# cloudflare/zkp-ecdsa

Measured on NVIDIA H100. Metric: ZKAttest proofs/sec, higher is better.
Workload: dtype u256/u258 (32-bit limbs, Montgomery)

## Files before the change

zkp_ecdsa_b200/csrc/zk_ops.cuh:

```cuda
#pragma once
#include "zk_curves.cuh"
#include "zk_layout.h"
#include "zk_sha256.cuh"

namespace zk {

#if defined(__CUDA_ARCH__)
#define ZK_SET_STATUS(ptr, code) atomicCAS((int*)(ptr), 0, (int)(code))
#define ZK_POST_MIN(ptr, key) atomicMin((int*)(ptr), (int)(key))
#define ZK_SET_STATUS_OVER(ptr, code, over) \
  do {                                      \
    atomicCAS((int*)(ptr), 0, (int)(code)); \
    atomicCAS((int*)(ptr), (int)(over), (int)(code)); \
  } while (0)
#else
#define ZK_SET_STATUS_OVER(ptr, code, over)              \
  do {                                                   \
    if (*(ptr) == 0 || *(ptr) == (over)) *(ptr) = (code); \
  } while (0)
#define ZK_SET_STATUS(ptr, code) \
  do {                           \
    if (*(ptr) == 0) *(ptr) = (code); \
  } while (0)
#define ZK_POST_MIN(ptr, key)             \
  do {                                    \
    if ((int)(key) < *(ptr)) *(ptr) = (int)(key); \
  } while (0)
#endif

template <int N>
ZK_HD void ld(uint32_t* r, const uint32_t* p) {
#pragma unroll
  for (int i = 0; i < N; i++) r[i] = p[i];
}
template <int N>
ZK_HD void st(uint32_t* p, const uint32_t* r) {
#pragma unroll
  for (int i = 0; i < N; i++) p[i] = r[i];
}

enum : int {
  P256_PROJ_WORDS = 24,
  P256_AFF_WORDS = 16,
#if defined(ZKA_PG_WAR256)
  TOM_PROJ_WORDS = 24,
  TOM_E2_WORDS = 24,
  TOM_AFF_WORDS = 16,
  TOM_PRE_WORDS = 16,
#else
  TOM_PROJ_WORDS = 28,
  TOM_E2_WORDS = 36,
  TOM_AFF_WORDS = 18,
  TOM_PRE_WORDS = 32,
#endif
  NORM_CHUNK_MAX = 64,
};


#if defined(ZKA_PG_WAR256)
ZK_HD void tom_st_xyz(uint32_t* m, const uint32_t* x, const uint32_t* y, const uint32_t* z) {
  st<8>(m, x); st<8>(m + 8, y); st<8>(m + 16, z);
}
ZK_HD void tom_ld_xyz(uint32_t* x, uint32_t* y, uint32_t* z, const uint32_t* m) {
  ld<8>(x, m); ld<8>(y, m + 8); ld<8>(z, m + 16);
}
ZK_HD void tom_ld_pre(TomPre& q, const uint32_t* m) { ld<8>(q.x, m); ld<8>(q.y, m + 8); }
#else
ZK_HD void tom_st_xyz(uint32_t* m, const uint32_t* x, const uint32_t* y, const uint32_t* z) {
  uint32_t w[28];
#pragma unroll
  for (int i = 0; i < 9; i++) { w[i] = x[i]; w[9 + i] = y[i]; w[18 + i] = z[i]; }
  w[27] = 0;
#if defined(__CUDA_ARCH__)
  uint4* v = reinterpret_cast<uint4*>(m);
#pragma unroll
  for (int i = 0; i < 7; i++) v[i] = make_uint4(w[4 * i], w[4 * i + 1], w[4 * i + 2], w[4 * i + 3]);
#else
  for (int i = 0; i < 28; i++) m[i] = w[i];
#endif
}
ZK_HD void tom_ld_xyz(uint32_t* x, uint32_t* y, uint32_t* z, const uint32_t* m) {
  uint32_t w[28];
#if defined(__CUDA_ARCH__)
  const uint4* v = reinterpret_cast<const uint4*>(m);
#pragma unroll
  for (int i = 0; i < 7; i++) {
    const uint4 u = v[i];
    w[4 * i] = u.x; w[4 * i + 1] = u.y; w[4 * i + 2] = u.z; w[4 * i + 3] = u.w;
  }
#else
  for (int i = 0; i < 28; i++) w[i] = m[i];
#endif
#pragma unroll
  for (int i = 0; i < 9; i++) { x[i] = w[i]; y[i] = w[9 + i]; z[i] = w[18 + i]; }
}
ZK_HD void tom_st_efgh(uint32_t* m, const TomEfgh& p) {
  uint32_t w[36];
#pragma unroll
  for (int i = 0; i < 9; i++) { w[i] = p.e[i]; w[9 + i] = p.f[i]; w[18 + i] = p.g[i]; w[27 + i] = p.h[i]; }
#if defined(__CUDA_ARCH__)
  uint4* v = reinterpret_cast<uint4*>(m);
#pragma unroll
  for (int i = 0; i < 9; i++) v[i] = make_uint4(w[4 * i], w[4 * i + 1], w[4 * i + 2], w[4 * i + 3]);
#else
  for (int i = 0; i < 36; i++) m[i] = w[i];
#endif
}
ZK_HD void tom_ld_efgh(uint32_t* e, uint32_t* f, uint32_t* g, uint32_t* h, const uint32_t* m) {
  uint32_t w[36];
#if defined(__CUDA_ARCH__)
  const uint4* v = reinterpret_cast<const uint4*>(m);
#pragma unroll
  for (int i = 0; i < 9; i++) {
    const uint4 u = v[i];
    w[4 * i] = u.x; w[4 * i + 1] = u.y; w[4 * i + 2] = u.z; w[4 * i + 3] = u.w;
  }
#else
  for (int i = 0; i < 36; i++) w[i] = m[i];
#endif
#pragma unroll
  for (int i = 0; i < 9; i++) { e[i] = w[i]; f[i] = w[9 + i]; g[i] = w[18 + i]; h[i] = w[27 + i]; }
}

ZK_HD void tom2_pre_neg(TomPre& q, bool neg) {
  uint32_t nk[9];
  Tomp::neg(nk, q.k);
#pragma unroll
  for (int i = 0; i < 9; i++) {
    const uint32_t a = q.x[i], b = q.y[i];
    q.x[i] = neg ? b : a;
    q.y[i] = neg ? a : b;
    q.k[i] = neg ? nk[i] : q.k[i];
  }
}
ZK_HD void tom_ld_pre(TomPre& q, const uint32_t* m) {
#if defined(__CUDA_ARCH__)
  const uint4* v = reinterpret_cast<const uint4*>(m);
  uint32_t w[32];
// ... 292 lines not shown
    TomPt p, acc;
    ld<9>(p.x, pow); ld<9>(p.y, pow + 9); ld<9>(p.t, pow + 18); ld<9>(p.z, pow + 27);
    const uint32_t* h = hi + (size_t)m * 36;
    ld<9>(acc.x, h); ld<9>(acc.y, h + 9); ld<9>(acc.t, h + 18); ld<9>(acc.z, h + 27);
    uint32_t* out = rows + ((size_t)m << 8) * TOM_PROJ_WORDS;
    const int n = m < nh ? 256 : 1;
    for (int d = 0; d < n; d++) {
      uint32_t* o = out + (size_t)d * TOM_PROJ_WORDS;
      tom_st_xyz(o, acc.x, acc.y, acc.z);
      tom_add(acc, acc, p);
    }
  }
};
struct TomTabE2Task {
  const uint32_t* proj;
  uint32_t* pre;
  int count;
  ZK_HD void operator()(int t) const {
    using F = Tomp;
    constexpr int CH = 16;
    const int lo = t * CH;
    int n = count - lo;
    if (n > CH) n = CH;
    if (n <= 0) return;
    uint32_t pf[CH][9];
    uint32_t acc[9], y[9], z[9], den[9];
    F::set_one(acc);
    for (int k = 0; k < n; k++) {
      const uint32_t* src = proj + (size_t)(lo + k) * TOM_PROJ_WORDS;
      uint32_t xx[9];
      tom_ld_xyz(xx, y, z, src);
      F::mul(den, y, z);
      F::mul(acc, acc, den);
      copy_n<9>(pf[k], acc);
    }
    uint32_t inv[9], s2[9], dd2[9];
    F::inv(inv, acc);
    tom_const(s2, TOM_SQRTND1);
    tom_const(dd2, TOM_2D2);
    for (int k = n - 1; k >= 0; k--) {
      const uint32_t* src = proj + (size_t)(lo + k) * TOM_PROJ_WORDS;
      uint32_t x[9], di[9], w[9], v[9], kk[9], ym[9], yp[9];
      tom_ld_xyz(x, y, z, src);
      F::mul(den, y, z);
      if (k > 0) F::mul(di, inv, pf[k - 1]); else copy_n<9>(di, inv);
      F::mul(inv, inv, den);
      F::mul(w, x, y);
      F::mul(w, w, di);
      F::mul(w, w, s2);
      F::sqr(v, z);
      F::mul(v, v, di);
      F::mul(kk, w, v);
      F::mul(kk, kk, dd2);
      F::sub(ym, v, w);
      F::add(yp, v, w);
      F::reduce(ym); F::reduce(yp); F::reduce(kk);
      uint32_t* o = pre + (size_t)(lo + k) * TOM_PRE_WORDS;
      st<9>(o, ym); st<9>(o + 9, yp); st<9>(o + 18, kk);
      for (int i = 27; i < 32; i++) o[i] = 0;
    }
  }
};

struct TomNormTask {
  const uint32_t* proj;
  uint32_t* aff;
  uint8_t* bytes;
  int count;
  int chunk;
  int e2;
  int aff_mod, aff_lim;
  int stride;
  ZK_HD static void canon2p(uint32_t* r) {
    uint32_t t[9], p2[9];
#pragma unroll
    for (int i = 0; i < 9; i++) p2[i] = (FpTom::p(i) << 1) | (i > 0 ? (FpTom::p(i - 1) >> 31) : 0u);
    uint32_t br = sub_n<9>(t, r, p2);
    csel_n<9>(r, br == 0, t, r);
    br = sub_p<FpTom>(t, r);
    csel_n<9>(r, br == 0, t, r);
  }
  ZK_HD void operator()(int t) const {
    using F = Tomp;
    const int lo = t * chunk;
    int n = count - lo;
    if (n > chunk) n = chunk;
    if (n <= 0) return;
    uint32_t pre[NORM_CHUNK_MAX][9];
    uint32_t acc[9], z[9], h[9], den[9];
    F::set_one(acc);
    for (int k = 0; k < n; k++) {
      const uint32_t* src = proj + (size_t)(lo + k) * stride;
      uint32_t xx[9], yy[9];
      if (e2) {
        tom_ld_efgh(xx, yy, z, h, src);
        F::mul(den, z, h);
      } else {
        tom_ld_xyz(xx, yy, den, src);
      }
      F::mul(acc, acc, den);
      copy_n<9>(pre[k], acc);
    }
    uint32_t inv[9], cxk[9], is2[9], one_plain[9];
    F::inv(inv, acc);
    tom_const(cxk, e2 ? TOM_INVSQRTND : TOM_INVSQRTA);
    tom_const(is2, TOM_INVSQRTND1);
    zero_n<9>(one_plain);
    one_plain[0] = 1;
    for (int k = n - 1; k >= 0; k--) {
      const uint32_t* src = proj + (size_t)(lo + k) * stride;
      uint32_t X[9], Y[9], di[9];
      if (e2) {
        tom_ld_efgh(X, Y, z, h, src);
        F::mul(den, z, h);
        F::mul(X, X, h);
        F::mul(Y, Y, z);
      } else {
        tom_ld_xyz(X, Y, den, src);
      }
      if (k > 0) F::mul(di, inv, pre[k - 1]); else copy_n<9>(di, inv);
      F::mul(inv, inv, den);
      if (bytes) {
        uint32_t Dp[9], cx[9], cy[9];
        F::mul(Dp, di, one_plain);
        F::mul(cx, X, cxk);
        F::mul(cx, cx, Dp);
        F::mul(cy, Y, Dp);
        canon2p(cx);
        canon2p(cy);
        store_point_words<9, 33>(bytes + (size_t)(lo + k) * BSTRIDE, 0x04u, cx, cy);
      }
      if (aff && ((lo + k) % aff_mod) < aff_lim) {
        uint32_t x[9], y[9];
        F::mul(x, X, di);
        if (e2) F::mul(x, x, is2);
        F::mul(y, Y, di);
        uint32_t* a = aff + (size_t)(lo + k) * TOM_AFF_WORDS;
        st<9>(a, x);
        st<9>(a + 9, y);
      }
    }
  }
};

ZK_HD void tom2_ld_entry(TomPre& q, const uint32_t* tab, const FbShape& sh, int j, uint32_t d, bool neg) {
  tom_ld_pre(q, tab + (sh.offset(j) + d) * TOM_PRE_WORDS);
  tom2_pre_neg(q, neg);
}

struct TomCommitTask {
  const uint32_t* jv;
  const uint32_t* jr;
  const uint32_t* gtab;
  const uint32_t* htab;
  uint32_t* proj;
  FbShape sh;
  int xyz = 0;
  ZK_HD void operator()(int t) const {
    uint32_t v[8], r[8];
    ld<8>(v, jv + (size_t)t * 8);
    ld<8>(r, jr + (size_t)t * 8);
    uint32_t cv = 0, cr = 0;
    bool nv, nr;
    TomPre q;
    uint32_t dv = signed_digit(v, 0, sh, cv, nv);
    tom2_ld_entry(q, gtab, sh, 0, dv, nv);
    TomPt acc;
    tom2_from_pre(acc, q);
    for (int j = 0;; j++) {
      const uint32_t dr = signed_digit(r, j, sh, cr, nr);
      tom2_ld_entry(q, htab, sh, j, dr, nr);
      if (j == sh.nwin - 1) break;
      tom2_madd<true>(acc, acc, q);
      dv = signed_digit(v, j + 1, sh, cv, nv);
      tom2_ld_entry(q, gtab, sh, j + 1, dv, nv);
      tom2_madd<true>(acc, acc, q);
    }
    if (xyz) {
      tom2_madd<false>(acc, acc, q);
      tom_st_xyz(proj + (size_t)t * TOM_PROJ_WORDS, acc.x, acc.y, acc.z);
    } else {
      TomEfgh e;
      tom2_madd_end(e, acc, q);
      tom_st_efgh(proj + (size_t)t * TOM_E2_WORDS, e);
    }
  }
};

struct TomCommitGTask {
  const uint32_t* jv;
  const uint32_t* gtab;
  uint32_t* ext;
  FbShape sh;
  GpartLayout lay;
  ZK_HD void operator()(int t) const {
    const int row = t / lay.gparts(), jb = lay.job_of_gpart(row, t % lay.gparts());
    if (jb < 0) return;
    uint32_t v[8];
    ld<8>(v, jv + ((size_t)row * lay.jobs() + jb) * 8);
    uint32_t carry = 0;
    bool neg;
    TomPre q;
    const uint32_t d0 = signed_digit(v, 0, sh, carry, neg);
    tom2_ld_entry(q, gtab, sh, 0, d0, neg);
    TomPt acc;
    tom2_from_pre<TompCommit>(acc, q);
#pragma unroll 1
    for (int j = 1; j < sh.nwin; j++) {
      const uint32_t d = signed_digit(v, j, sh, carry, neg);
      tom2_ld_entry(q, gtab, sh, j, d, neg);
      tom2_madd<true, TompCommit>(acc, acc, q);
    }
    uint32_t* o = ext + (size_t)t * TOM_EXT_WORDS;
    st<9>(o, acc.x); st<9>(o + 9, acc.y); st<9>(o + 18, acc.t); st<9>(o + 27, acc.z);
  }
};
struct TomCommitHTask {
  const uint32_t* jv;
  const uint32_t* jr;
  const uint32_t* gtab;
// ... 237 lines not shown
```

zkp_ecdsa_b200/csrc/zk_ops_war.cuh:

```cuda
#pragma once

#define WEI_PT WarPt
#define WEI_AFF WarAff
#define WEI_JAC WarJac
#define WEI_F Warp
#define WEI_FN(n) war_##n
#define WEI_T(n) War##n
#include "zk_weier_ops.inc"
#undef WEI_PT
#undef WEI_AFF
#undef WEI_JAC
#undef WEI_F
#undef WEI_FN
#undef WEI_T

struct TomNormTask {
  const uint32_t* proj;
  uint32_t* aff;
  uint8_t* bytes;
  int count;
  int chunk;
  int e2;
  int aff_mod, aff_lim;
  int stride;
  ZK_HD void operator()(int t) const {
    using F = Warp;
    const int lo = t * chunk;
    int n = count - lo;
    if (n > chunk) n = chunk;
    if (n <= 0) return;
    uint32_t pre[NORM_CHUNK_MAX][8];
    uint32_t acc[8], z[8], one[8];
    F::set_one(one);
    copy_n<8>(acc, one);
    for (int k = 0; k < n; k++) {
      ld<8>(z, proj + (size_t)(lo + k) * stride + 16);
      if (is_zero_n<8>(z)) copy_n<8>(z, one);
      F::mul(acc, acc, z);
      copy_n<8>(pre[k], acc);
    }
    uint32_t inv[8];
    F::inv(inv, acc);
    for (int k = n - 1; k >= 0; k--) {
      const uint32_t* src = proj + (size_t)(lo + k) * stride;
      ld<8>(z, src + 16);
      const bool isinf = is_zero_n<8>(z);
      if (isinf) copy_n<8>(z, one);
      uint32_t zi[8];
      if (k > 0) F::mul(zi, inv, pre[k - 1]); else copy_n<8>(zi, inv);
      F::mul(inv, inv, z);
      uint32_t X[8], Y[8], x[8], y[8];
      ld<8>(X, src);
      ld<8>(Y, src + 8);
      F::mul(x, X, zi);
      F::mul(y, Y, zi);
      if (aff && ((lo + k) % aff_mod) < aff_lim) {
        uint32_t* a = aff + (size_t)(lo + k) * TOM_AFF_WORDS;
        st<8>(a, x);
        st<8>(a + 8, y);
      }
      if (bytes) {
        uint32_t cx[8], cy[8];
        F::from_mont(cx, x);
        F::from_mont(cy, y);
        if (isinf) { zero_n<8>(cx); zero_n<8>(cy); }
        store_point_words<8, 32>(bytes + (size_t)(lo + k) * BSTRIDE, isinf ? 0x00u : 0x04u, cx, cy);
      }
    }
  }
};

struct TomCommitTask {
  const uint32_t* jv;
  const uint32_t* jr;
  const uint32_t* gtab;
  const uint32_t* htab;
  uint32_t* proj;
  FbShape sh;
  int xyz = 0;
  ZK_HD void operator()(int t) const {
    uint32_t v[8], r[8];
    ld<8>(v, jv + (size_t)t * 8);
    ld<8>(r, jr + (size_t)t * 8);
    WarJac aj;
    war_set_identity_jac(aj);
    war_accum_fixed_jac(aj, gtab, v, sh.w);
    war_accum_fixed_jac(aj, htab, r, sh.w);
    WarPt acc;
    war_jac_to_hom(acc, aj);
    war_st_proj(proj + (size_t)t * TOM_PROJ_WORDS, acc);
  }
};
ZK_HD void war_gpart(WarPt& acc, const uint32_t* gtab, const uint32_t* v, int w) {
  WarJac aj;
  war_set_identity_jac(aj);
  war_accum_fixed_jac(aj, gtab, v, w);
  war_jac_to_hom(acc, aj);
}
struct TomCommitGTask {
  const uint32_t* jv;
  const uint32_t* gtab;
  uint32_t* ext;
  FbShape sh;
  GpartLayout lay;
  ZK_HD void operator()(int t) const {
    const int row = t / lay.gparts(), jb = lay.job_of_gpart(row, t % lay.gparts());
    if (jb < 0) return;
    uint32_t v[8];
    ld<8>(v, jv + ((size_t)row * lay.jobs() + jb) * 8);
    WarPt acc;
    war_gpart(acc, gtab, v, sh.w);
    war_st_proj(ext + (size_t)t * TOM_EXT_WORDS, acc);
  }
};
struct TomCommitHTask {
  const uint32_t* jv;
  const uint32_t* jr;
  const uint32_t* gtab;
  const uint32_t* htab;
  const uint32_t* ext;
  uint32_t* proj;
  FbShape sh;
  GpartLayout lay;
  ZK_HD void operator()(int t) const {
    const int row = t / lay.jobs(), g = lay.gpart_of_job(row, t % lay.jobs());
    uint32_t v[8], r[8];
    ld<8>(v, jv + (size_t)t * 8);
    ld<8>(r, jr + (size_t)t * 8);
    WarPt acc;
    if (g < 0 || scalar_le_one(v)) war_gpart(acc, gtab, v, sh.w);
    else war_ld_proj(acc, ext + ((size_t)row * lay.gparts() + g) * TOM_EXT_WORDS);
    war_accum_fixed(acc, htab, r, sh.w);
    war_st_proj(proj + (size_t)t * TOM_PROJ_WORDS, acc);
  }
};
```

zkp_ecdsa_b200/csrc/zk_weier_ops.inc:

```
ZK_HD void WEI_FN(ld_proj)(WEI_PT& p, const uint32_t* m) {
  ld<8>(p.x, m); ld<8>(p.y, m + 8); ld<8>(p.z, m + 16);
}
ZK_HD void WEI_FN(st_proj)(uint32_t* m, const WEI_PT& p) {
  st<8>(m, p.x); st<8>(m + 8, p.y); st<8>(m + 16, p.z);
}
ZK_HD void WEI_FN(ld_aff)(WEI_AFF& a, const uint32_t* m) { ld<8>(a.x, m); ld<8>(a.y, m + 8); }
ZK_HD void WEI_FN(st_aff)(uint32_t* m, const WEI_AFF& a) { st<8>(m, a.x); st<8>(m + 8, a.y); }

struct WEI_T(PowsTask) {
  const uint32_t* base_aff;
  const uint8_t* base_inf;
  uint32_t* pows;
  int nbase, nwin, w;
  const uint32_t* index = nullptr;
  const uint32_t* count_dev = nullptr;
  const uint32_t* w_dev = nullptr;
  ZK_HD void operator()(int t) const {
    if (count_dev && (uint32_t)t >= *count_dev) return;
    const int w = w_dev ? (int)*w_dev : this->w;
    const int nwin = w_dev ? fb_windows(w) : this->nwin;
    const size_t src = index ? index[t] : (size_t)t;
    WEI_AFF a;
    WEI_FN(ld_aff)(a, base_aff + src * P256_AFF_WORDS);
    WEI_PT p;
// ... 20 lines not shown
    WEI_PT p, acc;
    WEI_FN(ld_proj)(p, pows + (size_t)t * P256_PROJ_WORDS);
    acc = p;
    const int ne = fb_entries(w);
    uint32_t* out = rows + (size_t)t * ne * P256_PROJ_WORDS;
    WEI_FN(st_proj)(out, p);
    for (int d = 1; d < ne; d++) {
      WEI_FN(st_proj)(out + (size_t)d * P256_PROJ_WORDS, acc);
      WEI_FN(add)(acc, acc, p);
    }
  }
};
struct WEI_T(RowsBlockTask) {
  const uint32_t* pows;
  uint32_t* rows;
  int w;
  const uint32_t* count_dev = nullptr;
  const uint32_t* w_dev = nullptr;
  ZK_HD void operator()(int t) const {
    const int w = w_dev ? (int)*w_dev : this->w;
    const int nblk = 1 << (w - 5), nwin = fb_windows(w);
    const int blk = t % nblk, bj = t / nblk;
    if (count_dev && (uint32_t)(bj / nwin) >= *count_dev) return;
    WEI_PT p, p16, acc;
    WEI_FN(ld_proj)(p, pows + (size_t)bj * P256_PROJ_WORDS);
    p16 = p;
    for (int i = 0; i < 4; i++) WEI_FN(dbl)(p16, p16);
    WEI_FN(set_identity)(acc);
    for (int bit = 2; bit >= 0; bit--) {
      WEI_FN(dbl)(acc, acc);
      if ((blk >> bit) & 1) WEI_FN(add)(acc, acc, p16);
    }
    uint32_t* out = rows + (size_t)bj * fb_entries(w) * P256_PROJ_WORDS;
    if (blk == 0) WEI_FN(st_proj)(out, p);
    for (int i = 1; i <= 16; i++) {
      WEI_FN(add)(acc, acc, p);
      WEI_FN(st_proj)(out + (size_t)(blk * 16 + i) * P256_PROJ_WORDS, acc);
    }
  }
};
struct WEI_T(RowsHiTask) {
  const uint32_t* pows;
  uint32_t* hi;
  uint32_t* rows;
  int w;
  ZK_HD void operator()(int t) const {
    WEI_PT p, acc;
    WEI_FN(ld_proj)(p, pows + (size_t)t * P256_PROJ_WORDS);
    for (int k = 0; k < 8; k++) WEI_FN(dbl)(p, p);
    WEI_FN(set_identity)(acc);
    const int nh = 1 << (w - 9);
    for (int m = 0; m < nh; m++) {
      WEI_FN(st_proj)(hi + ((size_t)t * nh + m) * P256_PROJ_WORDS, acc);
      WEI_FN(add)(acc, acc, p);
    }
    WEI_FN(st_proj)(rows + ((size_t)t * fb_entries(w) + ((size_t)1 << (w - 1))) * P256_PROJ_WORDS, acc);
  }
};
struct WEI_T(RowsLoTask) {
  const uint32_t* pows;
  const uint32_t* hi;
  uint32_t* rows;
  int w;
  ZK_HD void operator()(int t) const {
    const int nh = 1 << (w - 9);
    const int j = t / nh, m = t % nh;
    WEI_PT p, acc;
    WEI_FN(ld_proj)(p, pows + (size_t)j * P256_PROJ_WORDS);
    WEI_FN(ld_proj)(acc, hi + (size_t)t * P256_PROJ_WORDS);
    uint32_t* out = rows + ((size_t)j * fb_entries(w) + ((size_t)m << 8)) * P256_PROJ_WORDS;
    for (int d = 0; d < 256; d++) {
      WEI_FN(st_proj)(out + (size_t)d * P256_PROJ_WORDS, acc);
      WEI_FN(add)(acc, acc, p);
    }
  }
};

struct WEI_T(NormTask) {
  const uint32_t* proj;
  uint32_t* aff;
  uint8_t* bytes;
  uint8_t* inf;
  int count;
  int chunk;
  const uint32_t* groups_dev = nullptr;
  int group_size = 0;
  const uint32_t* w_dev = nullptr;
  ZK_HD void operator()(int t) const {
    using F = WEI_F;
    const int lo = t * chunk;
    int total = count;
    const int group_size = w_dev ? fb_windows((int)*w_dev) * fb_entries((int)*w_dev) : this->group_size;
    if (groups_dev) {
      const long long present = (long long)*groups_dev * group_size;
      if (present < total) total = (int)present;
    }
    int n = total - lo;
    if (n > chunk) n = chunk;
    if (n <= 0) return;
    uint32_t pre[NORM_CHUNK_MAX][8];
    uint32_t acc[8], z[8], one[8];
    F::set_one(one);
    copy_n<8>(acc, one);
    for (int k = 0; k < n; k++) {
      ld<8>(z, proj + (size_t)(lo + k) * P256_PROJ_WORDS + 16);
      if (is_zero_n<8>(z)) copy_n<8>(z, one);
      F::mul(acc, acc, z);
      copy_n<8>(pre[k], acc);
    }
    uint32_t inv[8];
    F::inv(inv, acc);
    for (int k = n - 1; k >= 0; k--) {
      const uint32_t* src = proj + (size_t)(lo + k) * P256_PROJ_WORDS;
      ld<8>(z, src + 16);
      const bool isinf = is_zero_n<8>(z);
      if (isinf) copy_n<8>(z, one);
      uint32_t zi[8];
      if (k > 0) F::mul(zi, inv, pre[k - 1]); else copy_n<8>(zi, inv);
      F::mul(inv, inv, z);
      WEI_AFF a;
      uint32_t X[8], Y[8];
      ld<8>(X, src);
      ld<8>(Y, src + 8);
      F::mul(a.x, X, zi);
      F::mul(a.y, Y, zi);
      WEI_FN(st_aff)(aff + (size_t)(lo + k) * P256_AFF_WORDS, a);
      if (inf) inf[lo + k] = isinf ? 1 : 0;
      if (bytes) {
        uint8_t* o = bytes + (size_t)(lo + k) * BSTRIDE;
        uint32_t cx[8], cy[8];
        F::from_mont(cx, a.x);
        F::from_mont(cy, a.y);
        if (isinf) { zero_n<8>(cx); zero_n<8>(cy); }
        store_point_words<8, 32>(o, isinf ? 0x00u : 0x04u, cx, cy);
      }
    }
  }
};

ZK_HD void WEI_FN(accum_fixed_jac)(WEI_JAC& acc, const uint32_t* tab, const uint32_t* k, int w) {
  const int nwin = fb_windows(w);
  const size_t E = (size_t)fb_entries(w);
  uint32_t carry = 0;
  for (int j = 0; j < nwin; j++) {
    bool neg;
    const uint32_t d = signed_digit(k, j, w, carry, neg);
    if (d) {
      WEI_AFF q;
      WEI_FN(ld_aff)(q, tab + ((size_t)j * E + d) * P256_AFF_WORDS);
      if (neg) WEI_F::neg(q.y, q.y);
      WEI_FN(jac_madd)(acc, acc, q);
    }
  }
}
ZK_HD void WEI_FN(accum_fixed)(WEI_PT& acc, const uint32_t* tab, const uint32_t* k, int w) {
  WEI_JAC q;
  WEI_FN(hom_to_jac)(q, acc);
  WEI_FN(accum_fixed_jac)(q, tab, k, w);
  WEI_FN(jac_to_hom)(acc, q);
}
ZK_HD void WEI_FN(set_identity_jac)(WEI_JAC& p) {
  WEI_F::set_one(p.x);
  WEI_F::set_one(p.y);
  zero_n<8>(p.z);
}
```

zkp_ecdsa_b200/csrc/zkattest.cu:

```cuda
#include "zkattest.h"

#include <math.h>
#include <stdio.h>

#include <algorithm>
#include <atomic>
#include <cmath>
#include <mutex>
#include <chrono>
#include <memory>
#include <thread>
#include <string>
#include <vector>

#include "zk_check.cuh"
#include "zk_launch.cuh"
#include "zk_prove.cuh"
#include "zk_seed.cuh"
#include "zk_verify_agg.cuh"

namespace zk {
struct ParsePointsTask {
  const uint8_t* nist;
  const uint8_t* tom;
// ... 292 lines not shown
  FixedTable gw;
  FixedTable tg;
  DevBuf tg_bytes;
  DevBuf lag;
  int lag_n = -1;
};

struct zka_params {
  zka_ctx* ctx = nullptr;
  uint32_t sec_level = 80;
  FixedTable h8;
  int h_w = 20;
  FixedTable th;
  uint8_t h_nist[65];
  uint8_t h_proof[WP];
  uint8_t hedge_digest[32];
};

struct zka_rings {
  zka_ctx* ctx = nullptr;
  uint32_t R = 0;
  std::vector<uint32_t> size;
  std::vector<int> depth;
  DevBuf ring_m, ring_base, ring_size, ring_depth;
  DevBuf lag;
  DevBuf ring_digest;
};

namespace {

int fail(zka_ctx* ctx, int code, const std::string& msg) {
  if (ctx) ctx->err = msg;
  return code;
}
template <class Fn>
int guarded(zka_ctx* ctx, Fn&& body) {
  try {
    return body();
  } catch (const std::exception& e) {
    return fail(ctx, ZKA_E_CUDA, e.what());
  }
}

template <class Src>
void agg_msm(Stream& st, Cursor A, const Src& src, const AggPlan& pl, const uint32_t* ctl, const uint32_t** rootA,
             const uint32_t** rootB) {
  const AggDigits& D = pl.D;
  const int nwin = D.nwin, nb = D.nb, nseg = (nb + 1 + AGG_SEG - 1) / AGG_SEG;
  const size_t cap = (size_t)src.slots();
  uint32_t* hist = A.take<uint32_t>((size_t)nwin * (nb + 1));
  uint32_t* bstart = A.take<uint32_t>((size_t)nwin * (nb + 2));
  uint32_t* segtot = A.take<uint32_t>((size_t)nwin * nseg);
  uint32_t* sorted = A.take<uint32_t>((size_t)nwin * cap);
  uint32_t* bsum = A.take<uint32_t>((size_t)nwin * nb * Src::PTW);
  dev_memset(st, hist, 0, (size_t)nwin * (nb + 1) * 4);
  launch(st, (long long)cap, AggHistTask<Src>{src, D, ctl, hist});
  launch(st, (long long)nwin * nseg, AggSegSumTask{ctl, hist, segtot, nb, nseg});
  launch(st, nwin, AggSegScanTask{ctl, segtot, nseg});
  launch(st, (long long)nwin * nseg, AggOffsetsTask{ctl, segtot, hist, bstart, nb, nseg});
  launch(st, (long long)cap, AggScatterTask<Src>{src, D, ctl, hist, sorted, cap});
  launch(st, (long long)nwin * nb, AggBucketTask<Src>{src, ctl, bstart, sorted, bsum, cap, nb});
  const uint32_t *inA = bsum, *inB = nullptr;
  int nin = nb, ll = 0;
  for (int lv = 0; lv < pl.levels; lv++) {
    const int nout = nin >> pl.lm[lv];
    uint32_t* oA = A.take<uint32_t>((size_t)nwin * nout * Src::PTW);
    uint32_t* oB = A.take<uint32_t>((size_t)nwin * nout * Src::PTW);
    launch(st, (long long)nwin * nout, AggLevelTask<Src>{ctl, inA, inB, oA, oB, nin, pl.lm[lv], ll, nwin, D.top_shift});
    inA = oA; inB = oB; nin = nout; ll += pl.lm[lv];
  }
  *rootA = inA;
  *rootB = inB;
}

int ceil_log2(uint32_t v) {
  int n = 0;
  while ((1ull << n) < v) n++;
  return n;
}


static int g_norm_slots = 132 * 4;
static bool g_norm_model = true;
inline int norm_chunk_for(long long count, int per_point = 11) {
  if (!g_norm_model) {
    long long c = count / 100000;
    if (c < 8) c = 8;
    if (c > NORM_CHUNK_MAX) c = NORM_CHUNK_MAX;
    return (int)c;
  }
  int best = 8;
  long long best_cost = -1;
  for (int c = 8; c <= NORM_CHUNK_MAX; c++) {
    const long long threads = (count + c - 1) / c, ctas = (threads + 127) / 128;
    const long long waves = (ctas + g_norm_slots - 1) / g_norm_slots;
    const long long cost = waves * ((long long)per_point * c + 70);
    if (best_cost < 0 || cost < best_cost) { best_cost = cost; best = c; }
  }
  return best;
}
inline void launch_p256_norm(Stream& st, const uint32_t* proj, uint32_t* aff, uint8_t* bytes, uint8_t* inf, long long count) {
  if (count <= 0) return;
  const int ch = norm_chunk_for(count, bytes ? 7 : 5);
  launch(st, (count + ch - 1) / ch, P256NormTask{proj, aff, bytes, inf, (int)count, ch});
}
inline void launch_tom_norm(Stream& st, const uint32_t* proj, uint32_t* aff, uint8_t* bytes, long long count, int e2,
                            int aff_mod = 1, int aff_lim = 1, int stride = 0) {
  if (count <= 0) return;
  const int ch = norm_chunk_for(count);
  if (stride == 0) stride = e2 ? TOM_E2_WORDS : TOM_PROJ_WORDS;
  launch(st, (count + ch - 1) / ch, TomNormTask{proj, aff, bytes, (int)count, ch, e2, aff_mod, aff_lim, stride});
}

void build_p256_tab(zka_ctx* ctx, const uint32_t* base_aff_dev, FixedTable& out, int w) {
  Stream& st = ctx->st;
  const int nwin = fb_windows(w);
  const size_t E = (size_t)fb_entries(w), count = (size_t)nwin * E;
  DevBuf pows, rows;
  uint32_t* d_pows = pows.get<uint32_t>((size_t)nwin * P256_PROJ_WORDS);
  uint32_t* d_rows = rows.get<uint32_t>(count * P256_PROJ_WORDS);
  out.tab = out.buf.get<uint32_t>(count * P256_AFF_WORDS);
  launch(st, 1, P256PowsTask{base_aff_dev, nullptr, d_pows, 1, nwin, w});
  if (w > 9) {
    DevBuf hi;
    const int nh = 1 << (w - 9);
    uint32_t* d_hi = hi.get<uint32_t>((size_t)nwin * nh * P256_PROJ_WORDS);
    launch(st, nwin, P256RowsHiTask{d_pows, d_hi, d_rows, w});
    launch(st, (long long)nwin * nh, P256RowsLoTask{d_pows, d_hi, d_rows, w});
    sync(st);
  } else {
    launch(st, nwin, P256RowsTask{d_pows, d_rows, w});
  }
  launch_p256_norm(st, d_rows, out.tab, nullptr, nullptr, (long long)(count));
  sync(st);
}
uint32_t* alloc_tom_tab(zka_ctx* ctx, DevBuf& buf) {
  const size_t words = ctx->tom.total() * TOM_PRE_WORDS;
  if (ctx->tom_table_max && words * sizeof(uint32_t) > ctx->tom_table_max)
    throw std::runtime_error("proof-group fixed-base table of " + std::to_string(words * sizeof(uint32_t)) + " bytes exceeds ZKA_TOM_TABLE_MAX");
  return buf.get_exact<uint32_t>(words);
}
#if defined(ZKA_PG_WAR256)
void build_tom_tab(zka_ctx* ctx, const uint32_t* base_aff_dev, FixedTable& out) {
  Stream& st = ctx->st;
  const int w = ctx->tom.w, nwin = ctx->tom.nwin;
  const size_t E = (size_t)fb_entries(w), count = (size_t)nwin * E;
  DevBuf pows, rows;
  uint32_t* d_pows = pows.get<uint32_t>((size_t)nwin * P256_PROJ_WORDS);
  uint32_t* d_rows = rows.get<uint32_t>(count * P256_PROJ_WORDS);
  out.tab = alloc_tom_tab(ctx, out.buf);
  launch(st, 1, WarPowsTask{base_aff_dev, nullptr, d_pows, 1, nwin, w});
  if (w > 9) {
    DevBuf hi;
    const int nh = 1 << (w - 9);
    uint32_t* d_hi = hi.get<uint32_t>((size_t)nwin * nh * P256_PROJ_WORDS);
    launch(st, nwin, WarRowsHiTask{d_pows, d_hi, d_rows, w});
    launch(st, (long long)nwin * nh, WarRowsLoTask{d_pows, d_hi, d_rows, w});
    sync(st);
  } else {
    launch(st, nwin, WarRowsTask{d_pows, d_rows, w});
  }
  {
    const int ch = norm_chunk_for((long long)count, 5);
    launch(st, ((long long)count + ch - 1) / ch, WarNormTask{d_rows, out.tab, nullptr, nullptr, (int)count, ch});
  }
  sync(st);
}
#else
void build_tom_tab(zka_ctx* ctx, const uint32_t* base_aff_dev, FixedTable& out) {
  Stream& st = ctx->st;
  const FbShape sh = ctx->tom;
  out.tab = alloc_tom_tab(ctx, out.buf);
  DevBuf pows, rows, hi;
  uint32_t* d_pows = pows.get<uint32_t>((size_t)sh.nwin * 36);
  uint32_t* d_rows = rows.get<uint32_t>(sh.entries(sh.nwin - 1) * TOM_PROJ_WORDS);
  launch(st, 1, TomPowsTask{base_aff_dev, d_pows, 1, sh});
  const bool two_level = sh.w > 9;
  uint32_t* d_hi = nullptr;
  if (two_level) {
    d_hi = hi.get<uint32_t>(tom_hi_offset(sh, sh.nwin) * 36);
    launch(st, sh.nwin, TomRowsHiTask{d_pows, d_hi, sh});
  }
  for (int j = 0; j < sh.nwin; j++) {
    const size_t ne = sh.entries(j);
    const uint32_t* pw = d_pows + (size_t)j * 36;
    if (two_level) {
      const int nh = 1 << (sh.width(j) - 9);
      launch(st, nh + 1, TomRowsLoTask{pw, d_hi + tom_hi_offset(sh, j) * 36, d_rows, nh});
    } else {
      launch(st, 1, TomRowsTask{pw, d_rows, sh.width(j)});
    }
    launch(st, (long long)(ne + 15) / 16, TomTabE2Task{d_rows, out.tab + sh.offset(j) * TOM_PRE_WORDS, (int)ne});
  }
  sync(st);
}

#endif

template <class T>
const T* stage_in(Stream& st, DevBuf& buf, const T* p, size_t count) {
  if (!p || count == 0) return p;
  if (is_device_ptr(p)) return p;
  T* d = buf.get<T>(count);
  copy_h2d(st, d, p, count * sizeof(T));
  return d;
}

template <class T>
struct Output {
  T* dst;
  size_t width;
  bool dev;
  Output(T* p, size_t width) : dst(p), width(width), dev(is_device_ptr(p)) {}
  T* rows(DevBuf& stage, uint32_t b0, size_t rows) const { return dev ? dst + b0 * width : stage.get<T>(rows * width); }
  void copy_back(Stream& st, uint32_t b0, const T* d, size_t rows) const {
    if (!dev) copy_d2h(st, dst + b0 * width, d, rows * width * sizeof(T));
  }
  void copy_back_2d(Stream& st, uint32_t b0, const T* d, size_t rows, size_t bytes) const {
    if (!dev) copy_d2h_2d(st, dst + b0 * width, width * sizeof(T), d, width * sizeof(T), bytes, rows);
  }
};

std::vector<uint32_t> chunk_schedule(uint32_t B, uint32_t cmax, int lanes, bool taper) {
  std::vector<uint32_t> off{0};
  auto r32 = [](uint32_t v) { return v < 32 ? std::max<uint32_t>(v, 1) : ((v + 31) & ~31u); };
  if (lanes > 1) {
    uint32_t per = r32((B + (uint32_t)lanes - 1) / (uint32_t)lanes);
    cmax = std::min(cmax, std::max<uint32_t>(per, 256));
  }
  uint32_t done = 0;
  auto push = [&](uint32_t n) { n = std::min(n, B - done); if (n) { done += n; off.push_back(done); } };
  if (taper && cmax >= 1024 && B >= 3 * cmax) {
    const uint32_t q = r32(cmax / 4), h = r32(cmax / 2);
    push(q);
    push(h);
    const uint32_t mid = B - done - (h + q);
    const uint32_t nm = (mid + cmax - 1) / cmax;
    const uint32_t each = r32((mid + nm - 1) / nm);
    for (uint32_t i = 0; i + 1 < nm; i++) push(each);
    push(B - done - (h + q));
    push(h);
    push(q);
  } else {
    const uint32_t nk = (B + cmax - 1) / cmax;
    const uint32_t each = r32((B + nk - 1) / nk);
    while (done < B) push(each);
  }
  return off;
// ... 1011 lines not shown
        d.tape = dt;
      }
      ev_record(ln.ev_tape[slot], ci);
    };
    uint32_t k = (uint32_t)li;
    int slot = 0;
    if (k < nchunks) issue_inputs(k, slot);
    for (; k < nchunks; slot ^= 1) {
      const uint32_t b0 = off[k];
      const int Bc = (int)(off[k + 1] - b0);
      const uint32_t k_this = k;
      const double t_begin = ms_now();
      ev_wait(st, ln.ev_small[slot]);
      ev_wait(st, ln.ev_out[slot]);
      ProveCtx c = prove_ctx(ctx, P, Bc, S, (int)ring.N, n);
      c.mode = mode; c.head_len = mode == 0 ? HEAD_LEN : 0;
      c.base = cin[slot].base; c.s_in = cin[slot].s_in; c.q_in = cin[slot].q_in;
      c.msg_hash = cin[slot].msg_hash;
      c.sig = cin[slot].sig;
      c.pk = cin[slot].pk;
      c.which = cin[slot].which;
      c.tape = cin[slot].tape;
      c.tape_stride = seeded ? (size_t)32 * seed_draws : is_device_ptr(rows.tape) ? rows.tape_stride : dev_tape_stride;
      c.tape_draws = seeded ? (uint32_t)seed_draws : (uint32_t)(rows.tape_stride / 32);
      ring.fill(c, ring_m, cin[slot].ring_of);
      const size_t S1 = (size_t)S + 1;
      const size_t nA = (size_t)Bc * S1;
      const size_t n1 = (size_t)Bc * (2 + 2 * S);
      Cursor w(ln.w);
      c.s1 = w.take<uint32_t>((size_t)Bc * 8);
      c.pk_aff = w.take<uint32_t>((size_t)Bc * 16);
      c.q_aff = w.take<uint32_t>((size_t)Bc * 16);
      c.q_inf = w.take<uint8_t>(Bc);
      c.r_aff = w.take<uint32_t>((size_t)Bc * 16);
      c.r_bytes = w.take<uint8_t>((size_t)Bc * BSTRIDE);
      c.rpows = w.take<uint32_t>((size_t)Bc * RT_NWIN * P256_PROJ_WORDS);
      c.rrows = w.take<uint32_t>((size_t)Bc * KEY_CAP * P256_PROJ_WORDS);
      c.rtab = w.take<uint32_t>((size_t)Bc * KEY_CAP * P256_AFF_WORDS);
      c.pa_T = w.take<uint32_t>(nA * P256_PROJ_WORDS);
      c.pa_A = w.take<uint32_t>(nA * P256_PROJ_WORDS);
      c.pa_T_aff = w.take<uint32_t>(nA * 16);
      c.pa_T_inf = w.take<uint8_t>(nA);
      c.pa_A_aff = w.take<uint32_t>(nA * 16);
      c.pa_A_bytes = w.take<uint8_t>(nA * BSTRIDE);
      c.pa_A_inf = w.take<uint8_t>(nA);
      c.s1_jv = w.take<uint32_t>(n1 * 8);
      c.s1_jr = w.take<uint32_t>(n1 * 8);
      c.s1_proj = w.take<uint32_t>(n1 * TOM_E2_WORDS);
      c.s1_aff = w.take<uint32_t>(n1 * TOM_AFF_WORDS);
      c.s1_bytes = w.take<uint8_t>(n1 * BSTRIDE);
      c.chal = w.take<uint32_t>((size_t)Bc * 3);
      c.zcount = w.take<uint32_t>(Bc);
      c.item_base = w.take<uint32_t>(Bc);
      c.item_total = w.take<uint32_t>(2);
      c.rep_off = w.take<uint32_t>((size_t)Bc * S);
      c.gk_off = w.take<uint32_t>(Bc);
      c.gk_dv = w.take<uint32_t>((size_t)Bc * n * 8);
      c.gk_x = w.take<uint32_t>((size_t)Bc * 3);
      c.u12 = w.take<uint32_t>((size_t)Bc * 16);
      c.tab_of = w.take<uint32_t>(Bc);
      c.tab_rep = w.take<uint32_t>((size_t)Bc * 2);
      c.tab_count = w.take<uint32_t>(2);
      c.which_s = w.take<uint32_t>(Bc);
      uint32_t* base_aff = w.take_if<uint32_t>(mode == 1, (size_t)Bc * 16);
      c.base_aff = mode == 0 ? c.pk_aff : base_aff;
      uint8_t* hedged = w.take_if<uint8_t>(hedge, (size_t)Bc * 32);
      const uint8_t* seeds = hedge ? hedged : cin[slot].seeds;
      c.proof_stride = rows.proof_stride;
      Cursor ob(ln.out[slot]);
      c.proofs = po.rows(ob.next(), b0, Bc);
      c.proof_len = lo.rows(ob.next(), b0, Bc);
      c.status = so.rows(ob.next(), b0, Bc);

      launch(st, Bc, PreKeyTask{c});
      launch(st, Bc, KeyDedupTask{c});
      launch(st, Bc, KeyRankTask{c});
      launch(st, Bc, KeyAssignTask{c});
      {
        const int Bp = (Bc + 31) & ~31;
        launch(st, (long long)Bp + Bc,
               PowsAndPreTask{P256PowsTask{c.base_aff, nullptr, c.rpows, Bc, RT_NWIN, RT_W, c.tab_rep, c.tab_count, c.tab_count + 1}, PreTask{c}, Bp});
      }
      launch(st, (long long)Bc * ((KEY_CAP + 15) / 16), P256RowsBlockTask{c.rpows, c.rrows, KEY_W_MIN, c.tab_count, c.tab_count + 1});
      {
        const long long np = (long long)Bc * KEY_CAP;
        const uint32_t kest = ring.set ? (uint32_t)Bc : std::min<uint32_t>(ring.N, (uint32_t)Bc);
        const int west = key_window_bits(kest, (uint32_t)Bc, (uint32_t)S + 2);
        const int ch = norm_chunk_for((long long)kest * fb_windows(west) * fb_entries(west), 5);
        launch(st, (np + ch - 1) / ch, P256NormTask{c.rrows, c.rtab, nullptr, nullptr, (int)np, ch, c.tab_count, 0, c.tab_count + 1});
      }
      ev_wait(st, ln.ev_tape[slot]);
      if (hedge) {
        SeedHedgeTask ht{{}, ring_digest, cin[slot].ring_of, cin[slot].seeds, c.msg_hash, c.sig, c.pk, c.which, hedged};
        memcpy(ht.params_digest, P->hedge_digest, 32);
        launch(st, Bc, ht);
      }
      if (seeded) {
        const int d1 = draws_before_items(S);
        launch(st, (long long)Bc * d1, SeedProveTapeTask{seeds, const_cast<uint8_t*>(c.tape), c.tape_stride, S, n, 0, d1, nullptr});
      }
      {
        const int nAp = (int)((nA + 31) & ~(size_t)31);
        launch(st, (long long)nAp + Bc, PhaseAAndRPointTask{PhaseAP256Task{c}, RPointTask{c}, (int)nA, nAp});
      }
      launch_p256_norm(st, c.pa_T, c.pa_T_aff, nullptr, c.pa_T_inf, (long long)(nA));
      launch_p256_norm(st, c.pa_A, c.pa_A_aff, c.pa_A_bytes, c.pa_A_inf, (long long)(nA));
      if (mode == 1) launch(st, Bc, ExpStatementTask{c});
      prove_store1(st, c);
      launch(st, Bc, ExpChallengeTask{c});
      launch(st, 1, ScanTask{c});
      uint32_t tot2[2] = {0, 0};
      copy_d2h(st, tot2, c.item_total, 8);
      const bool tape_host = !seeded && ctx->tape_split && !is_device_ptr(rows.tape);
      sync(st);
      if (seeded) {
        const int d1 = draws_before_items(S), span = prove_draws((int)tot2[1], n, S) - d1;
        launch(st, (long long)Bc * span,
               SeedProveTapeTask{seeds, const_cast<uint8_t*>(c.tape), c.tape_stride, S, n, d1, span, c.zcount, c.ring_of, c.ring_depth});
      } else if (tape_host) {
        const size_t o0 = (size_t)32 * draws_before_items(S);
        const size_t o1 = std::min(rows.tape_stride, (size_t)32 * prove_draws((int)tot2[1], n, S));
        if (o1 > o0)
          copy_d2h_2d(st, const_cast<uint8_t*>(c.tape) + o0, c.tape_stride, rows.at(b0).tape + o0, rows.tape_stride, o1 - o0, Bc);
      }
      const double t_mid = ms_now();
      {
        const uint32_t kn = next_chunk.fetch_add(1);
        if (kn < nchunks) issue_inputs(kn, slot ^ 1);
        k = kn;
      }
      const uint32_t M = tot2[0];
      const size_t max_len = mode == 0 ? (size_t)proof_len((int)tot2[1], n, S)
                                       : (size_t)tot2[1] * REP0_LEN + (size_t)(S - (int)tot2[1]) * REP1_LEN;
      c.M = (int)M;
      c.item_b = w.take<uint32_t>(M);
      c.item_i = w.take<uint32_t>(M);
      c.item_k = w.take<uint32_t>(M);
      c.pb_T1 = w.take<uint32_t>((size_t)M * P256_PROJ_WORDS);
      c.pb_T1_aff = w.take<uint32_t>((size_t)M * 16);
      c.pb_T1_inf = w.take<uint8_t>(M);
      const size_t n2 = c.s2_count();
      c.s2_jv = w.take<uint32_t>(n2 * 8);
      c.s2_jr = w.take<uint32_t>(n2 * 8);
      c.s2_proj = w.take<uint32_t>(n2 * TOM_E2_WORDS);
      c.s2_aff = w.take<uint32_t>(n2 * TOM_AFF_WORDS);
      c.s2_bytes = w.take<uint8_t>(n2 * BSTRIDE);
      c.secrets = w.take<uint32_t>((size_t)M * SECRETS_PER_ITEM * 8);
      c.item_inv = w.take<uint32_t>((size_t)M * 8);
      c.item_chal = w.take<uint32_t>((size_t)M * HASHES_PER_ITEM * 3);
      c.gk_part = w.take_if<uint32_t>(gk_blocks(n) > 1, (size_t)Bc * n * gk_blocks(n) * 8);
      uint32_t* gext = w.take<uint32_t>(prove_gext_words(c));
      launch(st, Bc, ItemsTask{c});
      launch(st, M, PhaseBP256Task{c});
      launch_p256_norm(st, c.pb_T1, c.pb_T1_aff, nullptr, c.pb_T1_inf, (long long)(M));
      prove_items_gk(st, c, gext, true, true);
      launch(st, (long long)nA, RepEmitTask{c});
      if (mode == 0) launch(st, Bc, GkEmitTask{c});
      launch(st, (long long)Bc * FIN_PARTS, FinalizeTask{c});
      if (check) {
        const uint8_t* key = seeded ? seeds : c.tape;
        check_chunk(ctx, P, ln, c, cin[slot], ring, ring_m, key, seeded ? 32 : c.tape_stride, seeded ? 32 : 96, b0, check_counts);
      }
      ev_record(ln.ev_done[slot], st);
      if (ctx->progress && k_this < ctx->progress_cap) notify_progress(st, ctx->progress + k_this);
      if (!po.dev || !lo.dev || !so.dev) {
        Stream& co = ln.cs_out;
        ev_wait(co, ln.ev_done[slot]);
        po.copy_back_2d(co, b0, c.proofs, Bc, max_len);
        lo.copy_back(co, b0, c.proof_len, Bc);
        so.copy_back(co, b0, c.status, Bc);
        ev_record(ln.ev_out[slot], co);
      }
      if (trace) {
// ... 685 lines not shown
```

Measured before the change: 122,100.

## Interleave batch-normalization chunks across warp lanes with fixed unrolled chunk size

Normalization tasks now assign points to threads in a warp-strided pattern, so lane j of a warp processes points first+32k. Adjacent lanes therefore touch adjacent points, which makes global loads and stores coalesced. The Weierstrass normalizers also switch from an adaptive chunk size to a fixed compile-time chunk of 16 with unrolled loops, so the prefix array can sit in registers instead of local memory. The tradeoffs are one field inversion per 16 points, which may be more inversions than the old model chose, plus higher register pressure from unrolling.

Result: no change. 123,100 (median of 6 runs) (+0.9%).

```diff
diff --git a/zkp_ecdsa_b200/csrc/zk_ops.cuh b/zkp_ecdsa_b200/csrc/zk_ops.cuh
--- a/zkp_ecdsa_b200/csrc/zk_ops.cuh
+++ b/zkp_ecdsa_b200/csrc/zk_ops.cuh
@@ -54,6 +54,18 @@
   TOM_PRE_WORDS = 32,
 #endif
   NORM_CHUNK_MAX = 64,
+  WEI_NORM_CHUNK = 16,
+};
+
+struct NormChunk {
+  int first, n;
+  ZK_HD NormChunk(int t, int count, int c) {
+    first = (t >> 5) * (32 * c) + (t & 31);
+    const int left = count - first;
+    n = left <= 0 ? 0 : ((left + 31) >> 5 < c ? (left + 31) >> 5 : c);
+  }
+  ZK_HD int at(int k) const { return first + 32 * k; }
+  static long long threads(long long count, int c) { return (count + 32LL * c - 1) / (32LL * c) * 32; }
 };
 
 
@@ -512,15 +524,14 @@
   }
   ZK_HD void operator()(int t) const {
     using F = Tomp;
-    const int lo = t * chunk;
-    int n = count - lo;
-    if (n > chunk) n = chunk;
-    if (n <= 0) return;
+    const NormChunk ch(t, count, chunk);
+    const int n = ch.n;
+    if (n == 0) return;
     uint32_t pre[NORM_CHUNK_MAX][9];
     uint32_t acc[9], z[9], h[9], den[9];
     F::set_one(acc);
     for (int k = 0; k < n; k++) {
-      const uint32_t* src = proj + (size_t)(lo + k) * stride;
+      const uint32_t* src = proj + (size_t)ch.at(k) * stride;
       uint32_t xx[9], yy[9];
       if (e2) {
         tom_ld_efgh(xx, yy, z, h, src);
@@ -538,7 +549,8 @@
     zero_n<9>(one_plain);
     one_plain[0] = 1;
     for (int k = n - 1; k >= 0; k--) {
-      const uint32_t* src = proj + (size_t)(lo + k) * stride;
+      const int i = ch.at(k);
+      const uint32_t* src = proj + (size_t)i * stride;
       uint32_t X[9], Y[9], di[9];
       if (e2) {
         tom_ld_efgh(X, Y, z, h, src);
@@ -558,14 +570,14 @@
         F::mul(cy, Y, Dp);
         canon2p(cx);
         canon2p(cy);
-        store_point_words<9, 33>(bytes + (size_t)(lo + k) * BSTRIDE, 0x04u, cx, cy);
+        store_point_words<9, 33>(bytes + (size_t)i * BSTRIDE, 0x04u, cx, cy);
       }
-      if (aff && ((lo + k) % aff_mod) < aff_lim) {
+      if (aff && (i % aff_mod) < aff_lim) {
         uint32_t x[9], y[9];
         F::mul(x, X, di);
         if (e2) F::mul(x, x, is2);
         F::mul(y, Y, di);
-        uint32_t* a = aff + (size_t)(lo + k) * TOM_AFF_WORDS;
+        uint32_t* a = aff + (size_t)i * TOM_AFF_WORDS;
         st<9>(a, x);
         st<9>(a + 9, y);
       }
diff --git a/zkp_ecdsa_b200/csrc/zk_ops_war.cuh b/zkp_ecdsa_b200/csrc/zk_ops_war.cuh
--- a/zkp_ecdsa_b200/csrc/zk_ops_war.cuh
+++ b/zkp_ecdsa_b200/csrc/zk_ops_war.cuh
@@ -19,30 +19,37 @@
   uint32_t* aff;
   uint8_t* bytes;
   int count;
-  int chunk;
   int e2;
   int aff_mod, aff_lim;
   int stride;
   ZK_HD void operator()(int t) const {
     using F = Warp;
-    const int lo = t * chunk;
-    int n = count - lo;
-    if (n > chunk) n = chunk;
-    if (n <= 0) return;
-    uint32_t pre[NORM_CHUNK_MAX][8];
+    const NormChunk ch(t, count, WEI_NORM_CHUNK);
+    if (ch.n == 0) return;
+    uint32_t pre[WEI_NORM_CHUNK][8];
     uint32_t acc[8], z[8], one[8];
     F::set_one(one);
     copy_n<8>(acc, one);
-    for (int k = 0; k < n; k++) {
-      ld<8>(z, proj + (size_t)(lo + k) * stride + 16);
+#pragma unroll
+    for (int k = 0; k < WEI_NORM_CHUNK; k++) {
+      if (k == ch.n) break;
+      ld<8>(z, proj + (size_t)ch.at(k) * stride + 16);
       if (is_zero_n<8>(z)) copy_n<8>(z, one);
       F::mul(acc, acc, z);
       copy_n<8>(pre[k], acc);
     }
     uint32_t inv[8];
-    F::inv(inv, acc);
-    for (int k = n - 1; k >= 0; k--) {
-      const uint32_t* src = proj + (size_t)(lo + k) * stride;
+    {
+      uint32_t a[8], r[8];
+      copy_n<8>(a, acc);
+      F::inv(r, a);
+      copy_n<8>(inv, r);
+    }
+#pragma unroll
+    for (int k = WEI_NORM_CHUNK - 1; k >= 0; k--) {
+      if (k >= ch.n) continue;
+      const int i = ch.at(k);
+      const uint32_t* src = proj + (size_t)i * stride;
       ld<8>(z, src + 16);
       const bool isinf = is_zero_n<8>(z);
       if (isinf) copy_n<8>(z, one);
@@ -54,8 +61,8 @@
       ld<8>(Y, src + 8);
       F::mul(x, X, zi);
       F::mul(y, Y, zi);
-      if (aff && ((lo + k) % aff_mod) < aff_lim) {
-        uint32_t* a = aff + (size_t)(lo + k) * TOM_AFF_WORDS;
+      if (aff && (i % aff_mod) < aff_lim) {
+        uint32_t* a = aff + (size_t)i * TOM_AFF_WORDS;
         st<8>(a, x);
         st<8>(a + 8, y);
       }
@@ -64,7 +71,7 @@
         F::from_mont(cx, x);
         F::from_mont(cy, y);
         if (isinf) { zero_n<8>(cx); zero_n<8>(cy); }
-        store_point_words<8, 32>(bytes + (size_t)(lo + k) * BSTRIDE, isinf ? 0x00u : 0x04u, cx, cy);
+        store_point_words<8, 32>(bytes + (size_t)i * BSTRIDE, isinf ? 0x00u : 0x04u, cx, cy);
       }
     }
   }
diff --git a/zkp_ecdsa_b200/csrc/zk_weier_ops.inc b/zkp_ecdsa_b200/csrc/zk_weier_ops.inc
--- a/zkp_ecdsa_b200/csrc/zk_weier_ops.inc
+++ b/zkp_ecdsa_b200/csrc/zk_weier_ops.inc
@@ -126,36 +126,43 @@
   uint8_t* bytes;
   uint8_t* inf;
   int count;
-  int chunk;
   const uint32_t* groups_dev = nullptr;
   int group_size = 0;
   const uint32_t* w_dev = nullptr;
   ZK_HD void operator()(int t) const {
     using F = WEI_F;
-    const int lo = t * chunk;
     int total = count;
     const int group_size = w_dev ? fb_windows((int)*w_dev) * fb_entries((int)*w_dev) : this->group_size;
     if (groups_dev) {
       const long long present = (long long)*groups_dev * group_size;
       if (present < total) total = (int)present;
     }
-    int n = total - lo;
-    if (n > chunk) n = chunk;
-    if (n <= 0) return;
-    uint32_t pre[NORM_CHUNK_MAX][8];
+    const NormChunk ch(t, total, WEI_NORM_CHUNK);
+    if (ch.n == 0) return;
+    uint32_t pre[WEI_NORM_CHUNK][8];
     uint32_t acc[8], z[8], one[8];
     F::set_one(one);
     copy_n<8>(acc, one);
-    for (int k = 0; k < n; k++) {
-      ld<8>(z, proj + (size_t)(lo + k) * P256_PROJ_WORDS + 16);
+#pragma unroll
+    for (int k = 0; k < WEI_NORM_CHUNK; k++) {
+      if (k == ch.n) break;
+      ld<8>(z, proj + (size_t)ch.at(k) * P256_PROJ_WORDS + 16);
       if (is_zero_n<8>(z)) copy_n<8>(z, one);
       F::mul(acc, acc, z);
       copy_n<8>(pre[k], acc);
     }
     uint32_t inv[8];
-    F::inv(inv, acc);
-    for (int k = n - 1; k >= 0; k--) {
-      const uint32_t* src = proj + (size_t)(lo + k) * P256_PROJ_WORDS;
+    {
+      uint32_t a[8], r[8];
+      copy_n<8>(a, acc);
+      F::inv(r, a);
+      copy_n<8>(inv, r);
+    }
+#pragma unroll
+    for (int k = WEI_NORM_CHUNK - 1; k >= 0; k--) {
+      if (k >= ch.n) continue;
+      const int i = ch.at(k);
+      const uint32_t* src = proj + (size_t)i * P256_PROJ_WORDS;
       ld<8>(z, src + 16);
       const bool isinf = is_zero_n<8>(z);
       if (isinf) copy_n<8>(z, one);
@@ -168,10 +175,10 @@
       ld<8>(Y, src + 8);
       F::mul(a.x, X, zi);
       F::mul(a.y, Y, zi);
-      WEI_FN(st_aff)(aff + (size_t)(lo + k) * P256_AFF_WORDS, a);
-      if (inf) inf[lo + k] = isinf ? 1 : 0;
+      WEI_FN(st_aff)(aff + (size_t)i * P256_AFF_WORDS, a);
+      if (inf) inf[i] = isinf ? 1 : 0;
       if (bytes) {
-        uint8_t* o = bytes + (size_t)(lo + k) * BSTRIDE;
+        uint8_t* o = bytes + (size_t)i * BSTRIDE;
         uint32_t cx[8], cy[8];
         F::from_mont(cx, a.x);
         F::from_mont(cy, a.y);
diff --git a/zkp_ecdsa_b200/csrc/zkattest.cu b/zkp_ecdsa_b200/csrc/zkattest.cu
--- a/zkp_ecdsa_b200/csrc/zkattest.cu
+++ b/zkp_ecdsa_b200/csrc/zkattest.cu
@@ -398,7 +398,7 @@
 
 static int g_norm_slots = 132 * 4;
 static bool g_norm_model = true;
-inline int norm_chunk_for(long long count, int per_point = 11) {
+inline int norm_chunk_for(long long count) {
   if (!g_norm_model) {
     long long c = count / 100000;
     if (c < 8) c = 8;
@@ -410,22 +410,24 @@
   for (int c = 8; c <= NORM_CHUNK_MAX; c++) {
     const long long threads = (count + c - 1) / c, ctas = (threads + 127) / 128;
     const long long waves = (ctas + g_norm_slots - 1) / g_norm_slots;
-    const long long cost = waves * ((long long)per_point * c + 70);
+    const long long cost = waves * (11LL * c + 70);
     if (best_cost < 0 || cost < best_cost) { best_cost = cost; best = c; }
   }
   return best;
 }
 inline void launch_p256_norm(Stream& st, const uint32_t* proj, uint32_t* aff, uint8_t* bytes, uint8_t* inf, long long count) {
-  if (count <= 0) return;
-  const int ch = norm_chunk_for(count, bytes ? 7 : 5);
-  launch(st, (count + ch - 1) / ch, P256NormTask{proj, aff, bytes, inf, (int)count, ch});
+  launch(st, NormChunk::threads(count, WEI_NORM_CHUNK), P256NormTask{proj, aff, bytes, inf, (int)count});
 }
 inline void launch_tom_norm(Stream& st, const uint32_t* proj, uint32_t* aff, uint8_t* bytes, long long count, int e2,
                             int aff_mod = 1, int aff_lim = 1, int stride = 0) {
   if (count <= 0) return;
+  if (stride == 0) stride = e2 ? TOM_E2_WORDS : TOM_PROJ_WORDS;
+#if defined(ZKA_PG_WAR256)
+  launch(st, NormChunk::threads(count, WEI_NORM_CHUNK), TomNormTask{proj, aff, bytes, (int)count, e2, aff_mod, aff_lim, stride});
+#else
   const int ch = norm_chunk_for(count);
-  if (stride == 0) stride = e2 ? TOM_E2_WORDS : TOM_PROJ_WORDS;
-  launch(st, (count + ch - 1) / ch, TomNormTask{proj, aff, bytes, (int)count, ch, e2, aff_mod, aff_lim, stride});
+  launch(st, NormChunk::threads(count, ch), TomNormTask{proj, aff, bytes, (int)count, ch, e2, aff_mod, aff_lim, stride});
+#endif
 }
 
 void build_p256_tab(zka_ctx* ctx, const uint32_t* base_aff_dev, FixedTable& out, int w) {
@@ -476,10 +478,7 @@
   } else {
     launch(st, nwin, WarRowsTask{d_pows, d_rows, w});
   }
-  {
-    const int ch = norm_chunk_for((long long)count, 5);
-    launch(st, ((long long)count + ch - 1) / ch, WarNormTask{d_rows, out.tab, nullptr, nullptr, (int)count, ch});
-  }
+  launch(st, NormChunk::threads((long long)count, WEI_NORM_CHUNK), WarNormTask{d_rows, out.tab, nullptr, nullptr, (int)count});
   sync(st);
 }
 #else
@@ -1657,13 +1656,8 @@
                PowsAndPreTask{P256PowsTask{c.base_aff, nullptr, c.rpows, Bc, RT_NWIN, RT_W, c.tab_rep, c.tab_count, c.tab_count + 1}, PreTask{c}, Bp});
       }
       launch(st, (long long)Bc * ((KEY_CAP + 15) / 16), P256RowsBlockTask{c.rpows, c.rrows, KEY_W_MIN, c.tab_count, c.tab_count + 1});
-      {
-        const long long np = (long long)Bc * KEY_CAP;
-        const uint32_t kest = ring.set ? (uint32_t)Bc : std::min<uint32_t>(ring.N, (uint32_t)Bc);
-        const int west = key_window_bits(kest, (uint32_t)Bc, (uint32_t)S + 2);
-        const int ch = norm_chunk_for((long long)kest * fb_windows(west) * fb_entries(west), 5);
-        launch(st, (np + ch - 1) / ch, P256NormTask{c.rrows, c.rtab, nullptr, nullptr, (int)np, ch, c.tab_count, 0, c.tab_count + 1});
-      }
+      launch(st, NormChunk::threads((long long)Bc * KEY_CAP, WEI_NORM_CHUNK),
+             P256NormTask{c.rrows, c.rtab, nullptr, nullptr, (int)((long long)Bc * KEY_CAP), c.tab_count, 0, c.tab_count + 1});
       ev_wait(st, ln.ev_tape[slot]);
       if (hedge) {
         SeedHedgeTask ht{{}, ring_digest, cin[slot].ring_of, cin[slot].seeds, c.msg_hash, c.sig, c.pk, c.which, hedged};
```
